# nanoporetech/scrappie

Measured on AMD Instinct MI355X. Metric: raw samples/sec, rgrgr_r94 4k-sample reads, higher is better.
Workload: dtype f32 (3xf16 split products, 22-bit operands, fp32 accumulate)

## Files before the change

include/scrappie_hip.h:

```cpp
#ifndef SCRAPPIE_HIP_H
#define SCRAPPIE_HIP_H

#include <stdbool.h>
#include <stddef.h>
#include <stdint.h>

#ifdef __cplusplus
extern "C" {
#endif


typedef struct {
    char *uuid;
    size_t n;
    size_t start;
    size_t end;
    float *raw;
} raw_table;

typedef struct {
    uint64_t start;
    float length;
    float mean;
    float stdv;
// ... 209 lines not shown

scrappie_matrix scrappie_hip_posterior(scrappie_hip_engine *e, int model, const raw_table signal,
                                       float min_prob, float tempW, float tempb, bool return_log);
scrappie_matrix scrappie_hip_trunk(scrappie_hip_engine *e, int model, const raw_table signal, int upto);

int scrappie_hip_event_features(const event_table events, float *out);
scrappie_matrix scrappie_hip_events_posterior(scrappie_hip_engine *e, int model, const float *feature3, size_t nevent,
                                              float min_prob, float tempW, float tempb, bool return_log);

long scrappie_hip_gru_schedule(const int *tile_T, size_t ntile, int ncu, int *nwg, int *capacity,
                               int *lane_off, int *seg, size_t cap);
long scrappie_hip_lane_schedule(const int *tile_T, size_t ntile, int ncu, int lanes_per_wg, int *nwg, int *capacity,
                                int *lane_off, int *seg, size_t cap);

long scrappie_hip_decoder_pieces(const int *tile_T, size_t ntile, int ncu, int *seg, size_t cap);

size_t scrappie_hip_min_samples(scrappie_hip_engine *e, int model);
int scrappie_hip_model_stride(scrappie_hip_engine *e, int model);
void scrappie_hip_set_profiling(scrappie_hip_engine *e, int on);
int scrappie_hip_get_timing(scrappie_hip_engine *e, scrappie_hip_timing *t);
void scrappie_hip_set_max_launch_reads(scrappie_hip_engine *e, size_t n);
void scrappie_hip_set_max_launch_blocks(scrappie_hip_engine *e, size_t n);
long scrappie_hip_plan_groups(const uint32_t *lengths, size_t n, int stride, size_t max_reads, size_t max_blocks,
                              size_t *starts, size_t cap);
unsigned scrappie_hip_host_thread_budget(void);
unsigned scrappie_hip_host_cpu_budget(void);
void *scrappie_hip_device_alloc(scrappie_hip_engine *e, size_t nbytes);
void scrappie_hip_device_free(scrappie_hip_engine *e, void *dptr);
int scrappie_hip_memcpy_h2d(scrappie_hip_engine *e, void *dst, const void *src, size_t nbytes);
int scrappie_hip_synchronize(scrappie_hip_engine *e);
// ... 18 lines not shown
```

scrappie_amd/csrc/scrappie_hip.hip:

```cpp
#include <hip/hip_runtime.h>
#include <sched.h>

#include <algorithm>
#include <atomic>
#include <cmath>
#include <cstdarg>
#include <cstdio>
#include <cstdlib>
#include <cstring>
#include <mutex>
#include <numeric>
#include <string>
#include <thread>
#include <vector>
#include <chrono>
#include <condition_variable>
#include <deque>
#include <map>
#include <memory>

#include "scrappie_hip.h"
#include "sh_internal.h"
#include "sh_kernels.h"
#include "sh_sched.h"
// ... 104 lines not shown
    std::vector<int> order;
    std::vector<int> rT, rN;
    std::vector<long long> seq_off, hp_off, bases_off;
    long long nbases_cap = 0;
    bool dev_stitch = false;
    bool dev_pos = false;
    int model = -1;
    bool hp_on = false;
    bool valid = false;
    int gru_nwg = 0;
    int gru1_nwg = 0;
    bool gru_two = false;
    int gru32_nwg = 0;
    int gru32x2_nwg = 0;
    int vit_nwg = 0;
    const float *d_signal = nullptr;
    std::vector<uint64_t> in_off;
    std::vector<uint32_t> in_len;
    scrappie_hip_params params{};
};

struct BatchReq {
    scrappie_hip_engine *e = nullptr;
    int model = 0;
    const raw_table *reads = nullptr;
    size_t n = 0;
    scrappie_hip_params p{};
    scrappie_hip_call *out = nullptr;
    int rc = -1;
    std::string err;
// ... 260 lines not shown
```

scrappie_amd/csrc/sh_decode.h:

```cpp
#ifndef SH_DECODE_H
#define SH_DECODE_H

struct ShVitArgs {
    const float *E;
    const float *sums;
    long long strideT;
    int strideQ, strideB;
    int want_log;
    float min_prob, stay_pen, skip_pen, local_pen;
    int use_slip;
    unsigned *tb;
    int *tb_end;
    int *final_state;
    float *final_score;
    float *hp_side;
    const long long *hp_off;
    unsigned long long *dbg;
    const ShGruSegD *seg;
    float *vstate;
    unsigned *flag;
    unsigned *err;
    int dump_final;
};

__device__ __forceinline__ void argmax_merge(float &v, int &i, float ov, int oi) {
    const bool take = (ov > v) | ((ov == v) & (oi < i));
    v = take ? ov : v;
    i = take ? oi : i;
}

__device__ __forceinline__ void rows_argmax(float &bv, int &bi) {
    float ov = __shfl_xor(bv, 16); int oi = __shfl_xor(bi, 16);
    argmax_merge(bv, bi, ov, oi);
// ... 949 lines not shown
```

scrappie_amd/csrc/sh_decode_teams.h:

```cpp
#ifndef SH_DECODE_TEAMS_H
#define SH_DECODE_TEAMS_H

#ifndef SH_FVT_WBUF
#define SH_FVT_WBUF 3
#endif
#ifndef SH_FVT_PROD_PRIO
#define SH_FVT_PROD_PRIO 1
#endif
#ifndef SH_FVT_ABL
#define SH_FVT_ABL 0
#endif
#ifndef SH_FVT_FLIP
#define SH_FVT_FLIP 3
#endif
#ifndef SH_FVT_STAMP
#ifdef SH_EXPERIMENTS
#define SH_FVT_STAMP 1
#else
#define SH_FVT_STAMP 0
#endif
#endif
#define SH_FVT_NTH 768
#define SH_FVT_LDS_FLOATS (1024 * 16 + 64 * 256 + 2 * 64 * 16 + 2 * 2 * 8 * 16 + 4 * 9 * 16 + 65 * 16 + 2 * 3 * 512 + 3 * 2 * 4 * 4)

template <bool SKIP0, bool DIV, bool NOCLAMP = false>
__global__ __launch_bounds__(SH_FVT_NTH) void k_ff_viterbi_teams(ShFfArgs f, ShVitArgs a, ShMeta md) {
    static_assert(!(DIV && NOCLAMP), "with temperatures the clamp stays");
    constexpr int NCW = 8, NPW = 4, PPT = 8, NQ = 256, NH = 1024, KS = 3, KQ = 6, TPP = 16, HT = 8, NG = 9, WB = SH_FVT_WBUF;
    static_assert(SH_SUM_GROUP == HT, "half a pass of a producer is one row-sum group");
    static_assert(WB >= 2 && WB <= 4, "weight ring");
    extern __shared__ __attribute__((aligned(16))) float smem[];
    float *sc = smem;
    float *ring = sc + NH * 16;
    float *skk = ring + 64 * 256;
    float *redv = skk + 2 * 64 * 16;
    int *redi = (int *)(redv + 2 * NCW * 16);
    float *gsum = (float *)(redi + 2 * NCW * 16);
    float *sBias = gsum + 4 * NG * 16;
    unsigned *xp = (unsigned *)(sBias + 65 * 16);
    unsigned *sStay = xp + 2 * KS * 512;

    const int tid = threadIdx.x, lane = tid & 63, b = lane & 15, q = lane >> 4;
    const int wave = __builtin_amdgcn_readfirstlane(tid >> 6);
    const bool decoder = wave < NCW;
    const float mp = a.min_prob, mpm1 = 1.0f - a.min_prob;
    const float lbound = (mp > 0.0f) ? 1.0e-3f - __logf(mp) : INFINITY;
    unsigned long long vA = 0, vB = 0, vC = 0, vD = 0, vt0 = 0, vt1 = 0;
    (void)vt0; (void)vt1;
#undef VSTAMP
#if SH_FVT_STAMP
#define VSTAMP(acc) do { if (a.dbg) { vt1 = __builtin_readcyclecounter(); acc += vt1 - vt0; vt0 = vt1; } } while (0)
#else
#define VSTAMP(acc) do { } while (0)
#endif

    if (tid < KS * 2 * 4 * 4) sStay[tid] = f.wpiece[(long long)(64) * KS * 512 + (tid >> 4) * 256 + ((tid >> 2) & 3) * 64 + (tid & 3)];
    for (int j = tid; j < 65 * 16; j += SH_FVT_NTH) sBias[j] = f.bfrag[((j >> 4) * 64 + ((j >> 2) & 3) * 16) * 4 + (j & 3)];

    int tile = blockIdx.x, s0 = 0, s1 = -1, ord = 0;
    if (a.seg) { const ShGruSegD sg = a.seg[blockIdx.x]; tile = sg.tile; s0 = sg.s0; s1 = sg.s1; ord = sg.pad; }
    tile = __builtin_amdgcn_readfirstlane(tile); s0 = __builtin_amdgcn_readfirstlane(s0); s1 = __builtin_amdgcn_readfirstlane(s1);
    const int Tt = __builtin_amdgcn_readfirstlane(md.tile_T[tile]);
    if (s1 < 0) s1 = Tt;
    const long long boff = __builtin_amdgcn_readfirstlane((int)md.tile_boff[tile]);
    const int rd = tile * 16 + b;
    int myT = md.rT[rd];
    asm volatile("" : "+v"(myT));
    const long long hpo = a.hp_side ? a.hp_off[rd] : 0;
    float pstart = 0.0f, pend = -SH_BIG;

    const int cw = decoder ? wave : 0;
    float *myq = sc + cw * 256 + lane * 4;
    const float *mye = ring + cw * 512 + lane * 4;
    const float *mysrc = sc + cw * 64 + b * 4 + q;
#define SH_FVT_MT(i) (16 * ((i) >> 1) + 8 * ((i) & 1))

    if (s0 == 0) {
        if (decoder) {
#pragma unroll
            for (int i = 0; i < PPT; i++) *(f32x4 *)(myq + SH_FVT_MT(i) * 256) = (f32x4){-SH_BIG, -SH_BIG, -SH_BIG, -SH_BIG};
            if (lane < 16) { redv[wave * 16 + b] = -SH_BIG - a.local_pen; redi[wave * 16 + b] = 4 * wave; }
        }
    } else {
        if (tid == 0) {
            if (!sh_wait_flag(a.flag + tile, (unsigned)ord, a.err)) __hip_atomic_store(a.err, 1u, __ATOMIC_RELAXED, __HIP_MEMORY_SCOPE_AGENT);
        }
        __syncthreads();
        __builtin_amdgcn_fence(__ATOMIC_ACQUIRE, "agent");
        if (decoder) {
            const float *vst = a.vstate + (long long)tile * (NH * 16 + 32);
            float bv = -INFINITY;
            int bi = 0x7fffffff;
#pragma unroll
            for (int i = 0; i < PPT; i++) {
                const int Q = 4 * (SH_FVT_MT(i) + cw) + q;
                const f32x4 pv = *(const f32x4 *)(vst + (Q * 16 + b) * 4);
                *(f32x4 *)(myq + SH_FVT_MT(i) * 256) = pv;
                {
                    const float ve = __builtin_fmaxf(__builtin_fmaxf(pv[0], pv[1]), __builtin_fmaxf(pv[2], pv[3])) - a.local_pen;
                    bi = (ve > bv) ? Q : bi;
                    bv = __builtin_fmaxf(bv, ve);
                }
            }
            pstart = vst[NH * 16 + b];
            pend = vst[NH * 16 + 16 + b];
// ... 149 lines not shown
            lds_barrier();
            VSTAMP(vD);
            if (more) w_prime(HT);
            VSTAMP(vA);
            lds_barrier();
            VSTAMP(vB);
            if (more) s1_half(H1, t + 2);
            __builtin_amdgcn_sched_barrier(0);
            xraw_load(t + 4);
            VSTAMP(vC);
            lds_barrier();
            VSTAMP(vD);
        }
        __syncthreads();
        if (s1 >= Tt) __syncthreads();
        if (a.dbg && lane == 0) { unsigned long long *d = a.dbg + ((long long)blockIdx.x * 12 + wave) * 8; d[0] = vA; d[1] = vB; d[2] = vC; d[3] = vD; d[4] = (unsigned long long)(s1 - s0); }
        return;
    }
    {
        f32x4 eN[2][PPT];
        auto drain = [&](auto a0, auto s0c, auto a1, auto s1c) {
            constexpr int A0 = decltype(a0)::value, S0 = decltype(s0c)::value, A1 = decltype(a1)::value, S1 = decltype(s1c)::value;
#pragma unroll
            for (int rl = 0; rl < PPT / 2; rl++) { eN[A0][2 * rl + S0] = *(const f32x4 *)(mye + rl * 4096); eN[A1][2 * rl + S1] = *(const f32x4 *)(mye + rl * 4096 + 256); }
        };
        const std::integral_constant<int, 0> I0{};
        const std::integral_constant<int, 1> I1{};
        __syncthreads();
        lds_barrier();
        lds_barrier();
        drain(I0, I0, I1, I0);
        lds_barrier();
        lds_barrier();
        if (a.dbg) vt0 = __builtin_readcyclecounter();
        const unsigned tofs = (unsigned)lane;
// ... 75 lines not shown
            const float rmf = d_rcp(tot) * mpm1;
            const float stay_lp = fin_log(gsum[((t & 3) * NG + NG - 1) * 16 + b], rmf, mp);
            const bool active = t < myT;
            const unsigned long long actmask = __builtin_amdgcn_ballot_w64(active);
            if (a.hp_side && active && tid < 16) (a.hp_side + (hpo + t) * 5)[4] = stay_lp;
            const float rm = active ? rmf : 0.0f;
            const float mpx = active ? mp : 0.0f;
            const float stay_v = active ? stay_lp - a.stay_pen : 0.0f;
            const float stay_act = stay_lp - a.stay_pen;
            const float hold = fmaxf(-a.local_pen, stay_act);
            const float nstart = pstart + hold;
            if (cw == 0) {
                float nend = pend + hold;
                const bool enter_end = ev > nend;
                nend = enter_end ? ev : nend;
                if (active && tid < 16) a.tb_end[cb * 16 + b] = enter_end ? tbe_in : NH + 1;
                if (active) pend = nend;
            }
            float bv = -INFINITY;
            int bi = 0x7fffffff;
            f32x4 pv_n; f32x2 kk_n;
            auto q_fetch = [&](int i) {
                pv_n = *(const f32x4 *)(myq + SH_FVT_MT(i) * 256);
                kk_n = *(const f32x2 *)(skk + ((SH_FVT_MT(i) + cw) * 16 + b) * 2);
            };
            q_fetch(0);
            float hpv[4] = {0.f, 0.f, 0.f, 0.f};
#pragma unroll
            for (int i = 0; i < PPT; i++) {
                const int QB = 4 * (SH_FVT_MT(i) + cw);
                const int Q = QB + q;
// ... 79 lines not shown
            }
            VSTAMP(vC);
            lds_barrier();
            VSTAMP(vD);
        };
        for (int t = s0; t < s1; t += 2) {
            block(t, std::true_type{});
            block(t + 1, std::false_type{});
#pragma unroll
            for (int rl = 0; rl < PPT / 2; rl++) eN[1][2 * rl] = eN[0][2 * rl + 1];
        }
    }

    if (s1 < Tt) {
        if (decoder) {
            float *vst = a.vstate + (long long)tile * (NH * 16 + 32);
#pragma unroll
            for (int i = 0; i < PPT; i++) {
                const int Q = 4 * (SH_FVT_MT(i) + cw) + q;
                *(f32x4 *)(vst + (Q * 16 + b) * 4) = *(const f32x4 *)(myq + SH_FVT_MT(i) * 256);
            }
            if (tid < 16) { vst[NH * 16 + b] = pstart; vst[NH * 16 + 16 + b] = pend; }
        }
        __builtin_amdgcn_fence(__ATOMIC_RELEASE, "agent");
        __syncthreads();
        if (tid == 0) __hip_atomic_store(a.flag + tile, (unsigned)ord + 1u, __ATOMIC_RELEASE, __HIP_MEMORY_SCOPE_AGENT);
    } else {
        float bv = -INFINITY;
        int bi = 0x7fffffff;
        if (decoder) {
#pragma unroll
            for (int i = 0; i < PPT; i++) {
                const int Q = 4 * (SH_FVT_MT(i) + cw) + q;
                const f32x4 pv = *(const f32x4 *)(myq + SH_FVT_MT(i) * 256);
#pragma unroll
                for (int k = 0; k < 4; k++) argmax_merge(bv, bi, pv[k], 4 * Q + k);
            }
            float ov = __shfl_xor(bv, 16); int oi = __shfl_xor(bi, 16);
            argmax_merge(bv, bi, ov, oi);
            ov = __shfl_xor(bv, 32); oi = __shfl_xor(bi, 32);
            argmax_merge(bv, bi, ov, oi);
        }
        __syncthreads();
        if (decoder && lane < 16) { redv[wave * 16 + b] = bv; redi[wave * 16 + b] = bi; }
        __syncthreads();
        if (tid < 16) {
            float ev = redv[b]; int ei = redi[b];
            for (int w = 1; w < NCW; w++) argmax_merge(ev, ei, redv[w * 16 + b], redi[w * 16 + b]);
            if (pstart > ev) { ev = pstart; ei = NH; }
            if (pend > ev) { ev = pend; ei = NH + 1; }
            a.final_state[rd] = ei;
            a.final_score[rd] = ev;
        }
        if (a.dump_final && a.vstate && decoder) {
            float *vst = a.vstate + (long long)tile * (NH * 16 + 32);
#pragma unroll
            for (int i = 0; i < PPT; i++) {
                const int Q = 4 * (SH_FVT_MT(i) + cw) + q;
                *(f32x4 *)(vst + (Q * 16 + b) * 4) = *(const f32x4 *)(myq + SH_FVT_MT(i) * 256);
            }
            if (tid < 16) { vst[NH * 16 + b] = pstart; vst[NH * 16 + 16 + b] = pend; }
        }
    }
    if (a.dbg && lane == 0) { unsigned long long *d = a.dbg + ((long long)blockIdx.x * 12 + wave) * 8; d[0] = vA; d[1] = vB; d[2] = vC; d[3] = vD; d[4] = (unsigned long long)(s1 - s0); }
#undef VSTAMP
#undef SH_FVT_MT
}

#endif
```

scrappie_amd/csrc/sh_eng_launch.inc:

```

struct MetaPtrs { ShMeta md; const long long *seq_off, *hp_off, *bases_off; ShGruLanes lanes, lanes1; ShGruPairs pairs, pairs2; const ShGruSegD *vseg; };

static int build_group(scrappie_hip_engine *e, Slot &sl, Model *m, const uint64_t *offsets, const uint32_t *lengths,
                       size_t n, bool hp_on, MetaPtrs &mp) {
    LaunchGroup &lg = sl.lg;
    lg.valid = false;
    lg.n = n; lg.hp_on = hp_on;
    lg.ntile = (n + 15) / 16; lg.npad = lg.ntile * 16;
    const int st = m->stride;
    std::vector<int> T(n);
    for (size_t i = 0; i < n; i++)
        T[i] = (lengths[i] >= m->min_samples) ? (int)((lengths[i] + st - 1) / st) : 0;
    lg.order.assign(lg.npad, -1);
    std::vector<int> idx(n);
    std::iota(idx.begin(), idx.end(), 0);
    std::stable_sort(idx.begin(), idx.end(), [&](int a, int b) { return T[a] > T[b]; });
    for (size_t i = 0; i < n; i++) lg.order[i] = idx[i];
    lg.rT.assign(lg.npad, 0); lg.rN.assign(lg.npad, 0);
    lg.seq_off.assign(lg.npad, 0); lg.hp_off.assign(lg.npad, 0); lg.bases_off.assign(lg.npad, 0);
    long long nbases = 0;
    const long long per_entry = (m->arch == 1) ? 1 : 5;
    std::vector<unsigned long long> sig_off(lg.npad, 0);
    std::vector<int> tile_T(lg.ntile, 0);
    std::vector<long long> tile_boff(lg.ntile, 0);
// ... 26 lines not shown
      if (e->dbg_gru_tiles == 1) lg.gru_two = false;
      if (e->dbg_gru_tiles == 2 && tmax < 65536) lg.gru_two = true; }
    std::vector<int> pair_tile, pair_T;
    for (size_t t = 0; t < lg.ntile; ) {
        const bool two = t + 1 < lg.ntile && tile_T[t] < (1 << 18) && tile_T[t + 1] > 0;
        pair_tile.push_back((int)t); pair_tile.push_back(two ? (int)t + 1 : -1);
        pair_T.push_back(std::max(tile_T[t], two ? tile_T[t + 1] : 0));
        t += two ? 2 : 1;
    }
    ShGruSchedule sched32;
    sh_lane_schedule(pair_T.data(), pair_T.size(), e->ncu, 1, sched32, e->handover);
    lg.gru32_nwg = sched32.nwg;
    ShGruSchedule sched32b;
    sh_lane_schedule(pair_T.data(), pair_T.size(), e->ncu, 2, sched32b, e->handover);
    lg.gru32x2_nwg = sched32b.nwg;
    std::vector<ShGruSeg> vseg;
    sh_piece_schedule(tile_T.data(), lg.ntile, e->ncu, vseg, e->handover);
    lg.vit_nwg = (int)vseg.size();
    const size_t b_u64 = lg.npad * 8, b_i32 = lg.npad * 4;
    const size_t b_loff = sched.lane_off.size() * 4, b_seg = sched.seg.size() * sizeof(ShGruSeg), b_wit = sched.wg_iter.size() * 4;
    const size_t b_vloff = 0, b_vseg = vseg.size() * sizeof(ShGruSeg);
    const size_t b_loff1 = sched1.lane_off.size() * 4, b_seg1 = sched1.seg.size() * sizeof(ShGruSeg);
    const size_t b_loff32 = sched32.lane_off.size() * 4, b_seg32 = sched32.seg.size() * sizeof(ShGruSeg), b_pt = pair_tile.size() * 4;
    const size_t b_loff32b = sched32b.lane_off.size() * 4, b_seg32b = sched32b.seg.size() * sizeof(ShGruSeg);
    const size_t total = 4 * b_u64 + lg.ntile * 8 + 2 * b_i32 + lg.ntile * 4 + 16 + b_seg + b_loff + b_wit + 16 + b_vseg + b_vloff + 16 + b_seg1 + b_loff1 +
                         16 + b_seg32 + b_loff32 + b_pt + 16 + b_seg32b + b_loff32b;
    if (sl.h_meta.ensure(total + 16) || sl.d_meta.ensure(total + 16)) return -1;
    char *h = sl.h_meta.as<char>();
    size_t o = 0;
    memcpy(h + o, sig_off.data(), b_u64); const size_t o_sig = o; o += b_u64;
    memcpy(h + o, lg.seq_off.data(), b_u64); const size_t o_seq = o; o += b_u64;
    memcpy(h + o, lg.hp_off.data(), b_u64); const size_t o_hp = o; o += b_u64;
    memcpy(h + o, lg.bases_off.data(), b_u64); const size_t o_bs = o; o += b_u64;
    memcpy(h + o, tile_boff.data(), lg.ntile * 8); const size_t o_tb = o; o += lg.ntile * 8;
    memcpy(h + o, lg.rN.data(), b_i32); const size_t o_n = o; o += b_i32;
    memcpy(h + o, lg.rT.data(), b_i32); const size_t o_t = o; o += b_i32;
    memcpy(h + o, tile_T.data(), lg.ntile * 4); const size_t o_tt = o; o += lg.ntile * 4;
    o = (o + 15) & ~(size_t)15;
    memcpy(h + o, sched.seg.data(), b_seg); const size_t o_seg = o; o += b_seg;
    memcpy(h + o, sched.lane_off.data(), b_loff); const size_t o_loff = o; o += b_loff;
    memcpy(h + o, sched.wg_iter.data(), b_wit); const size_t o_wit = o; o += b_wit;
    o = (o + 15) & ~(size_t)15;
    memcpy(h + o, vseg.data(), b_vseg); const size_t o_vseg = o; o += b_vseg;
    o = (o + 15) & ~(size_t)15;
    memcpy(h + o, sched1.seg.data(), b_seg1); const size_t o_seg1 = o; o += b_seg1;
    memcpy(h + o, sched1.lane_off.data(), b_loff1); const size_t o_loff1 = o; o += b_loff1;
    o = (o + 15) & ~(size_t)15;
    memcpy(h + o, sched32.seg.data(), b_seg32); const size_t o_seg32 = o; o += b_seg32;
    memcpy(h + o, sched32.lane_off.data(), b_loff32); const size_t o_loff32 = o; o += b_loff32;
    memcpy(h + o, pair_tile.data(), b_pt); const size_t o_pt = o; o += b_pt;
    o = (o + 15) & ~(size_t)15;
    memcpy(h + o, sched32b.seg.data(), b_seg32b); const size_t o_seg32b = o; o += b_seg32b;
    memcpy(h + o, sched32b.lane_off.data(), b_loff32b); const size_t o_loff32b = o; o += b_loff32b;
    hipStream_t ps = e->ev_ok ? e->pstream : e->stream;
    if (e->ev_ok) {
        const long long n16 = (long long)((total + 15) / 16);
        hipLaunchKernelGGL(k_upload_words, dim3((unsigned)std::min<long long>((n16 + 255) / 256, 64)), dim3(256), 0, ps, (const u32x4 *)h, sl.d_meta.as<u32x4>(), n16);
    } else HIPCHK(hipMemcpyAsync(sl.d_meta.p, h, total, hipMemcpyHostToDevice, ps));
    char *d = sl.d_meta.as<char>();
    mp.md.sig_off = (const unsigned long long *)(d + o_sig);
    mp.seq_off = (const long long *)(d + o_seq);
    mp.hp_off = (const long long *)(d + o_hp);
    mp.bases_off = (const long long *)(d + o_bs);
    mp.md.tile_boff = (const long long *)(d + o_tb);
    mp.md.rN = (const int *)(d + o_n);
    mp.md.rT = (const int *)(d + o_t);
    mp.md.tile_T = (const int *)(d + o_tt);
    static_assert(sizeof(ShGruSeg) == sizeof(ShGruSegD), "segment layout");
    mp.lanes.seg = (const ShGruSegD *)(d + o_seg);
    mp.lanes.lane_off = (const int *)(d + o_loff);
    mp.lanes.wg_iter = (const int *)(d + o_wit);
    mp.lanes.ntile = (int)lg.ntile;
    mp.vseg = (const ShGruSegD *)(d + o_vseg);
    if (e->d_hstate.ensure(std::max<size_t>(lg.ntile, 1) * 12 * 256 * 4) || sl.d_gflag.ensure((lg.ntile + 1) * 4)) return -1;
    mp.lanes.hstate = e->d_hstate.as<float>();
    mp.lanes.flag = sl.d_gflag.as<unsigned>();
    HIPCHK(hipMemsetAsync(sl.d_gflag.p, 0, (lg.ntile + 1) * 4, ps));
    if (sl.d_bad.ensure(lg.npad * 4)) return -1;
    HIPCHK(hipMemsetAsync(sl.d_bad.p, 0, lg.npad * 4, ps));
    mp.lanes1 = mp.lanes;
    mp.lanes1.seg = (const ShGruSegD *)(d + o_seg1);
    mp.lanes1.lane_off = (const int *)(d + o_loff1);
    mp.lanes1.wg_iter = nullptr;
    mp.pairs.seg = (const ShGruSegD *)(d + o_seg32);
    mp.pairs.lane_off = (const int *)(d + o_loff32);
    mp.pairs.pair_tile = (const int *)(d + o_pt);
    mp.pairs.hstate = mp.lanes.hstate;
    mp.pairs.flag = mp.lanes.flag;
// ... 650 lines not shown
    case 64: VIT_CASE(256, 1) break;
    case 256: VIT_CASE(256, 4) break;
    case 1024:
#ifdef SH_EXPERIMENTS
        if (getenv("SH_VIT_1024")) { VIT_CASE(1024, 4) break; }
#endif
        VIT_CASE(512, 8) break;
    default: return set_err("unsupported transducer state count %d (need 4^3, 4^4 or 4^5 k-mers)", NH);
    }
#undef VIT_CASE1
#undef VIT_CASE2
#undef VIT_CASE
    return 0;
}

static int launch_ff_viterbi(hipStream_t s, const ShFfArgs &f, const ShVitArgs &a, const ShMeta &md, size_t nwg, bool single) {
    const size_t lds = (size_t)SH_FV_LDS_FLOATS * 4;
    if (nwg == 0) return 0;
    dim3 grid((unsigned)nwg);
    if (!a.use_slip && !single) {
        const size_t ldt = (size_t)SH_FVT_LDS_FLOATS * 4;
#define FVT_CASE(SK0, DIV, NC)                                                                                    \
    {                                                                                                             \
        static DevOnce attr_once;                                                                                 \
        if (auto turn_ = attr_once.first())                                                                                    \
            HIPCHK(hipFuncSetAttribute((const void *)k_ff_viterbi_teams<SK0, DIV, NC>, hipFuncAttributeMaxDynamicSharedMemorySize, (int)ldt)); \
        hipLaunchKernelGGL((k_ff_viterbi_teams<SK0, DIV, NC>), grid, dim3(SH_FVT_NTH), ldt, s, f, a, md);         \
    }
        const bool skip0 = a.skip_pen == 0.0f, dv = f.out_div != 1.0f || f.in_div != 1.0f;
        static const bool keep_clamp = getenv("SH_FVT_KEEP_CLAMP") != nullptr;
        const bool nc = f.no_clamp && !dv && !keep_clamp;
        if (skip0) { if (dv) FVT_CASE(true, true, false) else if (nc) FVT_CASE(true, false, true) else FVT_CASE(true, false, false) }
        else { if (dv) FVT_CASE(false, true, false) else if (nc) FVT_CASE(false, false, true) else FVT_CASE(false, false, false) }
#undef FVT_CASE
        return 0;
    }
// ... 14 lines not shown
```

scrappie_amd/csrc/sh_eng_load.inc:

```

static const HostMat *find_mat(const std::vector<std::pair<std::string, HostMat>> &ms, const char *nm) {
    for (auto &kv : ms) if (kv.first == nm) return &kv.second;
    return nullptr;
}

static int load_model_mem_one(scrappie_hip_engine *e, const char *name, const void *blob, size_t nbytes);
extern "C" int scrappie_hip_load_model_mem(scrappie_hip_engine *e, const char *name, const void *blob, size_t nbytes) {
    const int idx = load_model_mem_one(e, name, blob, nbytes);
    if (idx < 0 || e->is_tail) return idx;
    scrappie_hip_engine::Blob b{name, std::vector<unsigned char>((const unsigned char *)blob, (const unsigned char *)blob + nbytes), e->dbg_force_f32};
    bool found = false;
    for (auto &x : e->blobs) if (x.name == b.name) { x = b; found = true; }
    if (!found) e->blobs.push_back(b);
    if (e->tail || e->tail2) {
        std::unique_lock<std::mutex> lk(e->tail_mu);
        e->tail_cv.wait(lk, [&] { return e->tail_busy == 0 && e->tail_q.empty(); });
    }
    for (scrappie_hip_engine **tp : {&e->tail, &e->tail2}) if (*tp) {
        (*tp)->dbg_force_f32 = e->dbg_force_f32;
        if (load_model_mem_one(*tp, name, blob, nbytes) != idx) return set_err("model '%s' did not load at the same index on the helper engine", name);
    }
    return idx;
}
static int load_model_mem_one(scrappie_hip_engine *e, const char *name, const void *blob, size_t nbytes) {
// ... 277 lines not shown
}

extern "C" long scrappie_hip_gru_schedule(const int *tile_T, size_t ntile, int ncu, int *nwg, int *capacity,
                                          int *lane_off, int *seg, size_t cap) {
    return scrappie_hip_lane_schedule(tile_T, ntile, ncu, 2, nwg, capacity, lane_off, seg, cap);
}

extern "C" long scrappie_hip_decoder_pieces(const int *tile_T, size_t ntile, int ncu, int *seg, size_t cap) {
    if (!tile_T || ncu < 1) return -1;
    std::vector<ShGruSeg> v;
    sh_piece_schedule(tile_T, ntile, ncu, v);
    if (seg) for (size_t i = 0; i < v.size() && i < cap; i++) memcpy(seg + 4 * i, &v[i], 16);
    return (long)v.size();
}

extern "C" long scrappie_hip_plan_groups(const uint32_t *lengths, size_t n, int stride, size_t max_reads, size_t max_blocks,
                                         size_t *starts, size_t cap) {
    if ((!lengths && n) || stride < 1 || max_reads < 1) return -1;
    long ng = 0;
    size_t cnt = 0;
    unsigned long long sumT = 0, maxT = 0;
    for (size_t i = 0; i < n; i++) {
        const unsigned long long T = ((unsigned long long)lengths[i] + stride - 1) / stride;
        if (max_blocks && T / 16 + T + 1 > max_blocks) return -1;
        const unsigned long long ns = sumT + T, nm = std::max(maxT, T);
        if (cnt == 0 || cnt >= max_reads || (max_blocks && ns / 16 + nm + 1 > max_blocks)) {
            if (starts && (size_t)ng < cap) starts[ng] = i;
            ng++;
            cnt = 0; sumT = 0; maxT = 0;
        }
// ... 25 lines not shown
```

scrappie_amd/csrc/sh_eng_pipeline.inc:

```

enum StopAt { STOP_NONE = 0, STOP_TRUNK = 1, STOP_POST = 2 };

struct RunOut {
    const float *act = nullptr;
    int act_units = 0;
    const float *E = nullptr;
    const float *sums = nullptr;
};

struct HostStamp {
    const std::chrono::steady_clock::time_point t0 = std::chrono::steady_clock::now();
    void operator()(const char *what, const char *after = "") const {
        if (tun().host_stamp) fprintf(stderr, "host stamp: %s %.2f ms%s\n", what, std::chrono::duration<double, std::milli>(std::chrono::steady_clock::now() - t0).count(), after);
    }
};

struct Marks {
    enum Mark { PROLOGUE_BEGIN, PROLOGUE_END,
                WAIT_BEGIN, MAIN_BEGIN,
                LAYER_BEGIN, LAYER_SPLIT, LAYER_END,
                S1_BEGIN, S1_END, DECODE_END, MAIN_END,
                WALK_BEGIN, WALK_END, STITCH_BEGIN, STITCH_END,
                N_MARKS };
    Slot *sl = nullptr;
// ... 242 lines not shown
    const int NH = m->NS - 1, NQ = NH / 4;
    if (e->d_tb.ensure((size_t)ncb * NQ * 16 * 4) || e->d_tbend.ensure((size_t)ncb * 16 * 4) || e->d_fstate.ensure(lg.npad * 4)) return -1;
    if (c.hp_on && sl.d_hp.ensure((size_t)std::max<long long>(lg.nhp, 1) * 5 * 4)) return -1;
    ShVitArgs va;
    va.E = E_use; va.sums = sums_use;
    va.strideT = (long long)mtiles * 256; va.strideQ = 64; va.strideB = 4;
    va.want_log = 1; va.min_prob = p->min_prob;
    va.stay_pen = p->stay_pen; va.skip_pen = p->skip_pen; va.local_pen = p->local_pen; va.use_slip = p->use_slip;
    va.tb = e->d_tb.as<unsigned>(); va.tb_end = e->d_tbend.as<int>();
    va.final_state = e->d_fstate.as<int>(); va.final_score = sl.d_fscore.as<float>();
    va.hp_side = c.hp_on ? sl.d_hp.as<float>() : nullptr; va.hp_off = mp.hp_off;
    va.dbg = nullptr;
    va.dump_final = e->dbg_dump_final ? 1 : 0;
    static unsigned long long *vdbg = nullptr;
    if (tun().vit_stamp) { if (!vdbg) (void)hipMalloc(&vdbg, 4096 * 16 * 8 * 8); va.dbg = vdbg; }
    if (e->d_vstate.ensure(std::max<size_t>(lg.ntile, 1) * ((size_t)NH * 16 + 32) * 4) || e->d_vflag.ensure(std::max<size_t>(lg.ntile, 1) * 4)) return -1;
    HIPCHK(hipMemsetAsync(e->d_vflag.p, 0, std::max<size_t>(lg.ntile, 1) * 4, s));
    va.seg = mp.vseg;
    va.vstate = e->d_vstate.as<float>(); va.flag = e->d_vflag.as<unsigned>(); va.err = sl.d_gflag.as<unsigned>() + lg.ntile;
    if (e->ev_ok && e->other(sl).pending) HIPCHK(hipStreamWaitEvent(s, e->other(sl).done, 0));
    if (fused) {
        ShFfArgs fa;
        fa.in = top; fa.wpiece = m->ffWp.as<unsigned>(); fa.bfrag = m->ffbs.as<float>();
        fa.in_div = p->tempW / p->tempb; fa.out_div = p->tempb;
        fa.no_clamp = (m->ff_no_clamp && !e->alt_trunk) ? 1 : 0;
        va.E = nullptr; va.sums = nullptr;
        if (launch_ff_viterbi(s, fa, va, mp.md, (size_t)lg.vit_nwg, tun().fv_single || e->dbg_fv_single)) return -1;
    } else if (launch_viterbi(s, NH, va, mp.md, (size_t)lg.vit_nwg)) return -1;
    if (va.dbg) {
        (void)sh_stream_wait(s);
        std::vector<unsigned long long> h((size_t)std::max(lg.vit_nwg, 1) * 16 * 8);
        (void)hipMemcpy(h.data(), vdbg, h.size() * 8, hipMemcpyDeviceToHost);
        const int nwv = (fused && !va.use_slip && !(tun().fv_single || e->dbg_fv_single)) ? 12 : 8;
        for (int w = 0; w < nwv; w++) { unsigned long long *d = &h[((size_t)(lg.vit_nwg / 2) * nwv + w) * 8]; fprintf(stderr, "vit stamp wave %d: phaseB %.0f bar %.0f phaseC %.0f bar %.0f cycles/block\n", w, d[0] / (double)d[4], d[1] / (double)d[4], d[2] / (double)d[4], d[3] / (double)d[4]); }
    }
    if (c.pf.mark(Marks::DECODE_END, s)) return -1;
    c.pf.span(F_DECODE, Marks::S1_END, Marks::DECODE_END);
    c.stamp("decoder enqueued at");
    c.walk_on_cs = e->ev_ok;
    if (c.walk_on_cs) { HIPCHK(hipEventRecord(sl.kdone, s)); HIPCHK(hipStreamWaitEvent(e->cstream, sl.kdone, 0)); }
    c.fold_tail = c.walk_on_cs && !tun().split_tail && !tun().host_stitch;
    if (!c.fold_tail) {
        hipStream_t bs = c.walk_on_cs ? e->cstream : s;
        if (c.pf.mark(Marks::WALK_BEGIN, bs)) return -1;
        hipLaunchKernelGGL(k_backtrace, dim3((unsigned)((lg.npad + 63) / 64)), dim3(64), 0, bs, e->d_tb.as<unsigned>(), e->d_tbend.as<int>(),
                           e->d_fstate.as<int>(), mp.md, mp.seq_off, sl.d_seq.as<int>(), (int)lg.npad, NQ, SH_SEQ_STRIDE);
        if (c.pf.mark(Marks::WALK_END, bs)) return -1;
        c.pf.span(F_BACKTRACE, Marks::WALK_BEGIN, Marks::WALK_END);
    }
// ... 143 lines not shown
```

scrappie_amd/csrc/sh_eng_surface.inc:

```

struct PostReq {
    int model = -1;
    raw_table sig{};
    float min_prob = 0.f, tempW = 1.f, tempb = 1.f;
    bool want_log = true;
    StopAt stop = STOP_POST;
    int upto = 5;
    scrappie_matrix out = nullptr;
    size_t nr = 0, nc = 0;
    const float *src = nullptr;
    size_t nbytes = 0;
    std::atomic<int> *users = nullptr;
    int phase = 0;
    char err[256] = "";
};
static void post_fail(PostReq *r, const char *fmt, ...) {
    va_list ap;
    va_start(ap, fmt);
    vsnprintf(r->err, sizeof r->err, fmt, ap);
    va_end(ap);
}
static void posterior_batch(scrappie_hip_engine *e, std::vector<PostReq *> &reqs) {
    if (reqs.empty()) return;
    Model *m = get_model(e, reqs[0]->model);
// ... 301 lines not shown
        char *d = dmeta.as<char>();
        ShMeta md;
        md.sig_off = (const unsigned long long *)d;
        md.tile_boff = (const long long *)(d + npad * 24);
        md.rN = (const int *)(d + npad * 24 + n * 8);
        md.rT = md.rN + npad;
        md.tile_T = md.rT + npad;
        ShVitArgs va;
        va.E = dpost.as<float>(); va.sums = nullptr;
        va.strideT = (long long)stride; va.strideQ = 4; va.strideB = 0;
        va.want_log = 0; va.min_prob = 0.f;
        va.stay_pen = f->stay_pen; va.skip_pen = f->skip_pen; va.local_pen = f->local_pen; va.use_slip = f->slip ? 1 : 0;
        va.tb = dtb.as<unsigned>(); va.tb_end = dtbe.as<int>();
        va.final_state = dfs.as<int>(); va.final_score = dfsc.as<float>();
        va.hp_side = nullptr; va.hp_off = nullptr; va.dbg = nullptr; va.dump_final = 0;
        va.seg = nullptr; va.vstate = nullptr; va.flag = nullptr; va.err = nullptr;
        if (launch_viterbi(s, NH, va, md, n)) break;
        hipLaunchKernelGGL(k_backtrace_lane0, dim3((unsigned)((n + 63) / 64)), dim3(64), 0, s, dtb.as<unsigned>(), dtbe.as<int>(), dfs.as<int>(), md,
                           (const long long *)(d + npad * 8), dseq.as<int>(), (int)n, NQ);
        int *hseq = e->h_dec_out.as<int>();
        if (hipMemcpyAsync(hseq, dseq.p, (size_t)nseq * 4, hipMemcpyDeviceToHost, s) != hipSuccess) break;
        if (hipMemcpyAsync(hseq + nseq, dfsc.p, npad * 4, hipMemcpyDeviceToHost, s) != hipSuccess) break;
        if (sh_stream_wait(s) != hipSuccess) break;
        const float *hsc = (const float *)(hseq + nseq);
        for (size_t k = 0; k < n; k++) {
            memcpy(reqs[k]->seq, hseq + seq_off[k * 16], ((size_t)reqs[k]->post->nc + 1) * 4);
            reqs[k]->score = hsc[k * 16];
        }
        ok = true;
    } while (0);
    if (!ok) { (void)hipGetLastError(); for (DecReq *r : reqs) r->score = NAN; }
// ... 160 lines not shown
```

scrappie_amd/csrc/sh_sched.h:

```cpp
#ifndef SH_SCHED_H
#define SH_SCHED_H
#include <algorithm>
#include <vector>

struct ShGruSeg { int tile, s0, s1, pad; };

struct ShGruSchedule {
    int nwg = 0;
    int capacity = 0;
    std::vector<int> lane_off;
    std::vector<ShGruSeg> seg;
    std::vector<int> wg_iter;
};

static inline void sh_lane_schedule(const int *tile_T, size_t ntile, int ncu, int lpw, ShGruSchedule &out,
                                    bool allow_split = true) {
    out = ShGruSchedule();
    std::vector<int> live;
    long long W = 0;
    int maxT = 0;
    for (size_t t = 0; t < ntile; t++) if (tile_T[t] > 0) { live.push_back((int)t); W += tile_T[t]; maxT = std::max(maxT, tile_T[t]); }
    if (live.empty()) { out.lane_off.assign(1, 0); return; }
    const long long nlive = (long long)live.size();
    const int nwg = (int)std::min<long long>(ncu, nlive);
// ... 38 lines not shown
    }
    out.nwg = nwg; out.capacity = M;
    out.lane_off.assign(L + 1, 0);
    out.wg_iter.assign(nwg, 0);
    for (int ln = 0; ln < L; ln++) {
        const std::vector<ShGruSeg> &v = pos[L - 1 - ln];
        int steps = 0;
        for (const ShGruSeg &sg : v) { out.seg.push_back(sg); steps += sg.s1 - sg.s0; }
        out.lane_off[ln + 1] = (int)out.seg.size();
        out.wg_iter[ln / lpw] = std::max(out.wg_iter[ln / lpw], steps);
    }
}
static inline void sh_gru_schedule(const int *tile_T, size_t ntile, int ncu, ShGruSchedule &out) {
    sh_lane_schedule(tile_T, ntile, ncu, 2, out);
}

static inline int sh_pieces_per_tile(long long nlive, int ncu) {
    if (nlive <= ncu) return 1;
    int best = 1;
    double bestv = 1e30;
    for (int k = 1; k <= 4; k++) {
        const double v = (double)((nlive * k + ncu - 1) / ncu) / k;
        if (v < bestv - 1e-9) { bestv = v; best = k; }
    }
    return best;
}
static inline void sh_piece_schedule(const int *tile_T, size_t ntile, int ncu, std::vector<ShGruSeg> &seg,
                                     bool allow_split = true) {
    seg.clear();
    long long nlive = 0;
// ... 13 lines not shown
```

Baseline: 1.582 billion.

## Make fused FF-Viterbi teams decoder persistent with per-CU lane schedule

```diff
diff --git a/include/scrappie_hip.h b/include/scrappie_hip.h
--- a/include/scrappie_hip.h
+++ b/include/scrappie_hip.h
@@ -247,6 +247,7 @@
                                 int *lane_off, int *seg, size_t cap);
 
 long scrappie_hip_decoder_pieces(const int *tile_T, size_t ntile, int ncu, int *seg, size_t cap);
+long scrappie_hip_decoder_lanes(const int *tile_T, size_t ntile, int ncu, int *nwg, int *capacity, int *lane_off, int *seg, size_t cap);
 
 size_t scrappie_hip_min_samples(scrappie_hip_engine *e, int model);
 int scrappie_hip_model_stride(scrappie_hip_engine *e, int model);
diff --git a/scrappie_amd/csrc/scrappie_hip.hip b/scrappie_amd/csrc/scrappie_hip.hip
--- a/scrappie_amd/csrc/scrappie_hip.hip
+++ b/scrappie_amd/csrc/scrappie_hip.hip
@@ -142,6 +142,7 @@
     int gru32_nwg = 0;
     int gru32x2_nwg = 0;
     int vit_nwg = 0;
+    int vit_npiece = 0;
     const float *d_signal = nullptr;
     std::vector<uint64_t> in_off;
     std::vector<uint32_t> in_len;
diff --git a/scrappie_amd/csrc/sh_decode.h b/scrappie_amd/csrc/sh_decode.h
--- a/scrappie_amd/csrc/sh_decode.h
+++ b/scrappie_amd/csrc/sh_decode.h
@@ -17,6 +17,7 @@
     const long long *hp_off;
     unsigned long long *dbg;
     const ShGruSegD *seg;
+    const int *lane_off;
     float *vstate;
     unsigned *flag;
     unsigned *err;
diff --git a/scrappie_amd/csrc/sh_decode_teams.h b/scrappie_amd/csrc/sh_decode_teams.h
--- a/scrappie_amd/csrc/sh_decode_teams.h
+++ b/scrappie_amd/csrc/sh_decode_teams.h
@@ -22,6 +22,8 @@
 #endif
 #define SH_FVT_NTH 768
 #define SH_FVT_LDS_FLOATS (1024 * 16 + 64 * 256 + 2 * 64 * 16 + 2 * 2 * 8 * 16 + 4 * 9 * 16 + 65 * 16 + 2 * 3 * 512 + 3 * 2 * 4 * 4)
+
+struct ShFvtKernArgs { ShFfArgs f; ShVitArgs a; ShMeta md; };
 
 template <bool SKIP0, bool DIV, bool NOCLAMP = false>
 __global__ __launch_bounds__(SH_FVT_NTH) void k_ff_viterbi_teams(ShFfArgs f, ShVitArgs a, ShMeta md) {
@@ -40,12 +42,13 @@
     unsigned *xp = (unsigned *)(sBias + 65 * 16);
     unsigned *sStay = xp + 2 * KS * 512;
 
-    const int tid = threadIdx.x, lane = tid & 63, b = lane & 15, q = lane >> 4;
-    const int wave = __builtin_amdgcn_readfirstlane(tid >> 6);
+    const int tid0 = threadIdx.x;
+    const int wave = __builtin_amdgcn_readfirstlane(tid0 >> 6);
     const bool decoder = wave < NCW;
     const float mp = a.min_prob, mpm1 = 1.0f - a.min_prob;
     const float lbound = (mp > 0.0f) ? 1.0e-3f - __logf(mp) : INFINITY;
     unsigned long long vA = 0, vB = 0, vC = 0, vD = 0, vt0 = 0, vt1 = 0;
+    int vblocks = 0;
     (void)vt0; (void)vt1;
 #undef VSTAMP
 #if SH_FVT_STAMP
@@ -54,26 +57,37 @@
 #define VSTAMP(acc) do { } while (0)
 #endif
 
-    if (tid < KS * 2 * 4 * 4) sStay[tid] = f.wpiece[(long long)(64) * KS * 512 + (tid >> 4) * 256 + ((tid >> 2) & 3) * 64 + (tid & 3)];
-    for (int j = tid; j < 65 * 16; j += SH_FVT_NTH) sBias[j] = f.bfrag[((j >> 4) * 64 + ((j >> 2) & 3) * 16) * 4 + (j & 3)];
-
-    int tile = blockIdx.x, s0 = 0, s1 = -1, ord = 0;
-    if (a.seg) { const ShGruSegD sg = a.seg[blockIdx.x]; tile = sg.tile; s0 = sg.s0; s1 = sg.s1; ord = sg.pad; }
-    tile = __builtin_amdgcn_readfirstlane(tile); s0 = __builtin_amdgcn_readfirstlane(s0); s1 = __builtin_amdgcn_readfirstlane(s1);
-    const int Tt = __builtin_amdgcn_readfirstlane(md.tile_T[tile]);
-    if (s1 < 0) s1 = Tt;
-    const long long boff = __builtin_amdgcn_readfirstlane((int)md.tile_boff[tile]);
-    const int rd = tile * 16 + b;
-    int myT = md.rT[rd];
-    asm volatile("" : "+v"(myT));
-    const long long hpo = a.hp_side ? a.hp_off[rd] : 0;
-    float pstart = 0.0f, pend = -SH_BIG;
-
+    if (tid0 < KS * 2 * 4 * 4) sStay[tid0] = f.wpiece[(long long)(64) * KS * 512 + (tid0 >> 4) * 256 + ((tid0 >> 2) & 3) * 64 + (tid0 & 3)];
+    for (int j = tid0; j < 65 * 16; j += SH_FVT_NTH) sBias[j] = f.bfrag[((j >> 4) * 64 + ((j >> 2) & 3) * 16) * 4 + (j & 3)];
+
+#define SH_FVT_MT(i) (16 * ((i) >> 1) + 8 * ((i) & 1))
+
+    int sgi = blockIdx.x, sgn = blockIdx.x + 1;
+    if (a.lane_off) { sgi = a.lane_off[blockIdx.x]; sgn = a.lane_off[blockIdx.x + 1]; }
+    sgi = __builtin_amdgcn_readfirstlane(sgi); sgn = __builtin_amdgcn_readfirstlane(sgn);
+    auto segment = [&](auto dec_c, const int sgi) __attribute__((always_inline)) {
+    constexpr bool decoder = decltype(dec_c)::value;
     const int cw = decoder ? wave : 0;
+    typedef const __attribute__((address_space(4))) ShFvtKernArgs *kargs_t;
+    kargs_t ka = (kargs_t)__builtin_amdgcn_kernarg_segment_ptr();
+    asm volatile("" : "+s"(ka));
+    int lane;
+    asm volatile("v_mbcnt_lo_u32_b32 %0, -1, 0\n\tv_mbcnt_hi_u32_b32 %0, -1, %0" : "=v"(lane));
+    const int tid = wave * 64 + lane, b = lane & 15, q = lane >> 4;
     float *myq = sc + cw * 256 + lane * 4;
     const float *mye = ring + cw * 512 + lane * 4;
     const float *mysrc = sc + cw * 64 + b * 4 + q;
-#define SH_FVT_MT(i) (16 * ((i) >> 1) + 8 * ((i) & 1))
+    int tile = sgi, s0 = 0, s1 = -1, ord = 0;
+    if (ka->a.seg) { const ShGruSegD sg = ka->a.seg[sgi]; tile = sg.tile; s0 = sg.s0; s1 = sg.s1; ord = sg.pad; }
+    tile = __builtin_amdgcn_readfirstlane(tile); s0 = __builtin_amdgcn_readfirstlane(s0); s1 = __builtin_amdgcn_readfirstlane(s1);
+    const int Tt = __builtin_amdgcn_readfirstlane(ka->md.tile_T[tile]);
+    if (s1 < 0) s1 = Tt;
+    const long long boff = __builtin_amdgcn_readfirstlane((int)ka->md.tile_boff[tile]);
+    const int rd = tile * 16 + b;
+    int myT = ka->md.rT[rd];
+    asm volatile("" : "+v"(myT));
+    const long long hpo = a.hp_side ? ka->a.hp_off[rd] : 0;
+    float pstart = 0.0f, pend = -SH_BIG;
 
     if (s0 == 0) {
         if (decoder) {
@@ -83,12 +97,12 @@
         }
     } else {
         if (tid == 0) {
-            if (!sh_wait_flag(a.flag + tile, (unsigned)ord, a.err)) __hip_atomic_store(a.err, 1u, __ATOMIC_RELAXED, __HIP_MEMORY_SCOPE_AGENT);
+            if (!sh_wait_flag(ka->a.flag + tile, (unsigned)ord, ka->a.err)) __hip_atomic_store(ka->a.err, 1u, __ATOMIC_RELAXED, __HIP_MEMORY_SCOPE_AGENT);
         }
         __syncthreads();
         __builtin_amdgcn_fence(__ATOMIC_ACQUIRE, "agent");
         if (decoder) {
-            const float *vst = a.vstate + (long long)tile * (NH * 16 + 32);
+            const float *vst = ka->a.vstate + (long long)tile * (NH * 16 + 32);
             float bv = -INFINITY;
             int bi = 0x7fffffff;
 #pragma unroll
@@ -268,11 +282,12 @@
         }
         __syncthreads();
         if (s1 >= Tt) __syncthreads();
-        if (a.dbg && lane == 0) { unsigned long long *d = a.dbg + ((long long)blockIdx.x * 12 + wave) * 8; d[0] = vA; d[1] = vB; d[2] = vC; d[3] = vD; d[4] = (unsigned long long)(s1 - s0); }
+        vblocks += s1 - s0;
+        __syncthreads();
         return;
     }
     {
-        f32x4 eN[2][PPT];
+        f32x4 eN[2][PPT] = {};
         auto drain = [&](auto a0, auto s0c, auto a1, auto s1c) {
             constexpr int A0 = decltype(a0)::value, S0 = decltype(s0c)::value, A1 = decltype(a1)::value, S1 = decltype(s1c)::value;
 #pragma unroll
@@ -378,7 +393,11 @@
                 float nend = pend + hold;
                 const bool enter_end = ev > nend;
                 nend = enter_end ? ev : nend;
-                if (active && tid < 16) a.tb_end[cb * 16 + b] = enter_end ? tbe_in : NH + 1;
+                if (active && tid < 16) {
+                    unsigned bo = (unsigned)b;
+                    asm volatile("" : "+v"(bo));
+                    (a.tb_end + cb * 16)[bo] = enter_end ? tbe_in : NH + 1;
+                }
                 if (active) pend = nend;
             }
             float bv = -INFINITY;
@@ -488,7 +507,7 @@
 
     if (s1 < Tt) {
         if (decoder) {
-            float *vst = a.vstate + (long long)tile * (NH * 16 + 32);
+            float *vst = ka->a.vstate + (long long)tile * (NH * 16 + 32);
 #pragma unroll
             for (int i = 0; i < PPT; i++) {
                 const int Q = 4 * (SH_FVT_MT(i) + cw) + q;
@@ -498,7 +517,7 @@
         }
         __builtin_amdgcn_fence(__ATOMIC_RELEASE, "agent");
         __syncthreads();
-        if (tid == 0) __hip_atomic_store(a.flag + tile, (unsigned)ord + 1u, __ATOMIC_RELEASE, __HIP_MEMORY_SCOPE_AGENT);
+        if (tid == 0) __hip_atomic_store(ka->a.flag + tile, (unsigned)ord + 1u, __ATOMIC_RELEASE, __HIP_MEMORY_SCOPE_AGENT);
     } else {
         float bv = -INFINITY;
         int bi = 0x7fffffff;
@@ -523,11 +542,11 @@
             for (int w = 1; w < NCW; w++) argmax_merge(ev, ei, redv[w * 16 + b], redi[w * 16 + b]);
             if (pstart > ev) { ev = pstart; ei = NH; }
             if (pend > ev) { ev = pend; ei = NH + 1; }
-            a.final_state[rd] = ei;
-            a.final_score[rd] = ev;
-        }
-        if (a.dump_final && a.vstate && decoder) {
-            float *vst = a.vstate + (long long)tile * (NH * 16 + 32);
+            ka->a.final_state[rd] = ei;
+            ka->a.final_score[rd] = ev;
+        }
+        if (ka->a.dump_final && ka->a.vstate && decoder) {
+            float *vst = ka->a.vstate + (long long)tile * (NH * 16 + 32);
 #pragma unroll
             for (int i = 0; i < PPT; i++) {
                 const int Q = 4 * (SH_FVT_MT(i) + cw) + q;
@@ -536,7 +555,12 @@
             if (tid < 16) { vst[NH * 16 + b] = pstart; vst[NH * 16 + 16 + b] = pend; }
         }
     }
-    if (a.dbg && lane == 0) { unsigned long long *d = a.dbg + ((long long)blockIdx.x * 12 + wave) * 8; d[0] = vA; d[1] = vB; d[2] = vC; d[3] = vD; d[4] = (unsigned long long)(s1 - s0); }
+    vblocks += s1 - s0;
+    __syncthreads();
+    };
+    if (decoder) { for (; sgi < sgn; sgi++) segment(std::true_type{}, sgi); }
+    else { for (; sgi < sgn; sgi++) segment(std::false_type{}, sgi); }
+    if (a.dbg && __builtin_amdgcn_mbcnt_hi(~0u, __builtin_amdgcn_mbcnt_lo(~0u, 0u)) == 0) { unsigned long long *d = a.dbg + ((long long)blockIdx.x * 12 + wave) * 8; d[0] = vA; d[1] = vB; d[2] = vC; d[3] = vD; d[4] = (unsigned long long)vblocks; }
 #undef VSTAMP
 #undef SH_FVT_MT
 }
diff --git a/scrappie_amd/csrc/sh_eng_launch.inc b/scrappie_amd/csrc/sh_eng_launch.inc
--- a/scrappie_amd/csrc/sh_eng_launch.inc
+++ b/scrappie_amd/csrc/sh_eng_launch.inc
@@ -1,5 +1,5 @@
 
-struct MetaPtrs { ShMeta md; const long long *seq_off, *hp_off, *bases_off; ShGruLanes lanes, lanes1; ShGruPairs pairs, pairs2; const ShGruSegD *vseg; };
+struct MetaPtrs { ShMeta md; const long long *seq_off, *hp_off, *bases_off; ShGruLanes lanes, lanes1; ShGruPairs pairs, pairs2; const ShGruSegD *vseg, *vlseg; const int *vlane_off; };
 
 static int build_group(scrappie_hip_engine *e, Slot &sl, Model *m, const uint64_t *offsets, const uint32_t *lengths,
                        size_t n, bool hp_on, MetaPtrs &mp) {
@@ -64,16 +64,19 @@
     ShGruSchedule sched32b;
     sh_lane_schedule(pair_T.data(), pair_T.size(), e->ncu, 2, sched32b, e->handover);
     lg.gru32x2_nwg = sched32b.nwg;
+    ShGruSchedule vsched;
+    sh_decoder_lanes(tile_T.data(), lg.ntile, e->ncu, vsched, e->handover);
+    lg.vit_nwg = vsched.nwg;
     std::vector<ShGruSeg> vseg;
     sh_piece_schedule(tile_T.data(), lg.ntile, e->ncu, vseg, e->handover);
-    lg.vit_nwg = (int)vseg.size();
+    lg.vit_npiece = (int)vseg.size();
     const size_t b_u64 = lg.npad * 8, b_i32 = lg.npad * 4;
     const size_t b_loff = sched.lane_off.size() * 4, b_seg = sched.seg.size() * sizeof(ShGruSeg), b_wit = sched.wg_iter.size() * 4;
-    const size_t b_vloff = 0, b_vseg = vseg.size() * sizeof(ShGruSeg);
+    const size_t b_vseg = vseg.size() * sizeof(ShGruSeg), b_vloff = vsched.lane_off.size() * 4, b_vlseg = vsched.seg.size() * sizeof(ShGruSeg);
     const size_t b_loff1 = sched1.lane_off.size() * 4, b_seg1 = sched1.seg.size() * sizeof(ShGruSeg);
     const size_t b_loff32 = sched32.lane_off.size() * 4, b_seg32 = sched32.seg.size() * sizeof(ShGruSeg), b_pt = pair_tile.size() * 4;
     const size_t b_loff32b = sched32b.lane_off.size() * 4, b_seg32b = sched32b.seg.size() * sizeof(ShGruSeg);
-    const size_t total = 4 * b_u64 + lg.ntile * 8 + 2 * b_i32 + lg.ntile * 4 + 16 + b_seg + b_loff + b_wit + 16 + b_vseg + b_vloff + 16 + b_seg1 + b_loff1 +
+    const size_t total = 4 * b_u64 + lg.ntile * 8 + 2 * b_i32 + lg.ntile * 4 + 16 + b_seg + b_loff + b_wit + 16 + b_vseg + b_vlseg + b_vloff + 16 + b_seg1 + b_loff1 +
                          16 + b_seg32 + b_loff32 + b_pt + 16 + b_seg32b + b_loff32b;
     if (sl.h_meta.ensure(total + 16) || sl.d_meta.ensure(total + 16)) return -1;
     char *h = sl.h_meta.as<char>();
@@ -92,6 +95,8 @@
     memcpy(h + o, sched.wg_iter.data(), b_wit); const size_t o_wit = o; o += b_wit;
     o = (o + 15) & ~(size_t)15;
     memcpy(h + o, vseg.data(), b_vseg); const size_t o_vseg = o; o += b_vseg;
+    memcpy(h + o, vsched.seg.data(), b_vlseg); const size_t o_vlseg = o; o += b_vlseg;
+    memcpy(h + o, vsched.lane_off.data(), b_vloff); const size_t o_vloff = o; o += b_vloff;
     o = (o + 15) & ~(size_t)15;
     memcpy(h + o, sched1.seg.data(), b_seg1); const size_t o_seg1 = o; o += b_seg1;
     memcpy(h + o, sched1.lane_off.data(), b_loff1); const size_t o_loff1 = o; o += b_loff1;
@@ -122,6 +127,8 @@
     mp.lanes.wg_iter = (const int *)(d + o_wit);
     mp.lanes.ntile = (int)lg.ntile;
     mp.vseg = (const ShGruSegD *)(d + o_vseg);
+    mp.vlseg = (const ShGruSegD *)(d + o_vlseg);
+    mp.vlane_off = (const int *)(d + o_vloff);
     if (e->d_hstate.ensure(std::max<size_t>(lg.ntile, 1) * 12 * 256 * 4) || sl.d_gflag.ensure((lg.ntile + 1) * 4)) return -1;
     mp.lanes.hstate = e->d_hstate.as<float>();
     mp.lanes.flag = sl.d_gflag.as<unsigned>();
@@ -802,12 +809,13 @@
     return 0;
 }
 
-static int launch_ff_viterbi(hipStream_t s, const ShFfArgs &f, const ShVitArgs &a, const ShMeta &md, size_t nwg, bool single) {
+static int launch_ff_viterbi(hipStream_t s, const ShFfArgs &f, const ShVitArgs &a, const ShMeta &md, size_t nwg, bool single, int ncu) {
     const size_t lds = (size_t)SH_FV_LDS_FLOATS * 4;
     if (nwg == 0) return 0;
     dim3 grid((unsigned)nwg);
     if (!a.use_slip && !single) {
         const size_t ldt = (size_t)SH_FVT_LDS_FLOATS * 4;
+        if (a.lane_off && nwg > (size_t)ncu) return set_err("decoder: %zu persistent workgroups for %d CUs", nwg, ncu);
 #define FVT_CASE(SK0, DIV, NC)                                                                                    \
     {                                                                                                             \
         static DevOnce attr_once;                                                                                 \
diff --git a/scrappie_amd/csrc/sh_eng_load.inc b/scrappie_amd/csrc/sh_eng_load.inc
--- a/scrappie_amd/csrc/sh_eng_load.inc
+++ b/scrappie_amd/csrc/sh_eng_load.inc
@@ -315,6 +315,18 @@
     return (long)v.size();
 }
 
+extern "C" long scrappie_hip_decoder_lanes(const int *tile_T, size_t ntile, int ncu, int *nwg, int *capacity, int *lane_off,
+                                           int *seg, size_t cap) {
+    if (!tile_T || ncu < 1) return -1;
+    ShGruSchedule sc;
+    sh_decoder_lanes(tile_T, ntile, ncu, sc);
+    if (nwg) *nwg = sc.nwg;
+    if (capacity) *capacity = sc.capacity;
+    if (lane_off) memcpy(lane_off, sc.lane_off.data(), sc.lane_off.size() * sizeof(int));
+    if (seg) for (size_t i = 0; i < sc.seg.size() && i < cap; i++) memcpy(seg + 4 * i, &sc.seg[i], 16);
+    return (long)sc.seg.size();
+}
+
 extern "C" long scrappie_hip_plan_groups(const uint32_t *lengths, size_t n, int stride, size_t max_reads, size_t max_blocks,
                                          size_t *starts, size_t cap) {
     if ((!lengths && n) || stride < 1 || max_reads < 1) return -1;
diff --git a/scrappie_amd/csrc/sh_eng_pipeline.inc b/scrappie_amd/csrc/sh_eng_pipeline.inc
--- a/scrappie_amd/csrc/sh_eng_pipeline.inc
+++ b/scrappie_amd/csrc/sh_eng_pipeline.inc
@@ -280,9 +280,12 @@
     va.dump_final = e->dbg_dump_final ? 1 : 0;
     static unsigned long long *vdbg = nullptr;
     if (tun().vit_stamp) { if (!vdbg) (void)hipMalloc(&vdbg, 4096 * 16 * 8 * 8); va.dbg = vdbg; }
+    const bool teams = fused && !va.use_slip && !(tun().fv_single || e->dbg_fv_single);
+    const int vit_nwg = teams ? lg.vit_nwg : lg.vit_npiece;
     if (e->d_vstate.ensure(std::max<size_t>(lg.ntile, 1) * ((size_t)NH * 16 + 32) * 4) || e->d_vflag.ensure(std::max<size_t>(lg.ntile, 1) * 4)) return -1;
     HIPCHK(hipMemsetAsync(e->d_vflag.p, 0, std::max<size_t>(lg.ntile, 1) * 4, s));
-    va.seg = mp.vseg;
+    va.seg = teams ? mp.vlseg : mp.vseg;
+    va.lane_off = teams ? mp.vlane_off : nullptr;
     va.vstate = e->d_vstate.as<float>(); va.flag = e->d_vflag.as<unsigned>(); va.err = sl.d_gflag.as<unsigned>() + lg.ntile;
     if (e->ev_ok && e->other(sl).pending) HIPCHK(hipStreamWaitEvent(s, e->other(sl).done, 0));
     if (fused) {
@@ -291,14 +294,14 @@
         fa.in_div = p->tempW / p->tempb; fa.out_div = p->tempb;
         fa.no_clamp = (m->ff_no_clamp && !e->alt_trunk) ? 1 : 0;
         va.E = nullptr; va.sums = nullptr;
-        if (launch_ff_viterbi(s, fa, va, mp.md, (size_t)lg.vit_nwg, tun().fv_single || e->dbg_fv_single)) return -1;
-    } else if (launch_viterbi(s, NH, va, mp.md, (size_t)lg.vit_nwg)) return -1;
+        if (launch_ff_viterbi(s, fa, va, mp.md, (size_t)vit_nwg, !teams, e->ncu)) return -1;
+    } else if (launch_viterbi(s, NH, va, mp.md, (size_t)vit_nwg)) return -1;
     if (va.dbg) {
         (void)sh_stream_wait(s);
-        std::vector<unsigned long long> h((size_t)std::max(lg.vit_nwg, 1) * 16 * 8);
+        std::vector<unsigned long long> h((size_t)std::max(vit_nwg, 1) * 16 * 8);
         (void)hipMemcpy(h.data(), vdbg, h.size() * 8, hipMemcpyDeviceToHost);
-        const int nwv = (fused && !va.use_slip && !(tun().fv_single || e->dbg_fv_single)) ? 12 : 8;
-        for (int w = 0; w < nwv; w++) { unsigned long long *d = &h[((size_t)(lg.vit_nwg / 2) * nwv + w) * 8]; fprintf(stderr, "vit stamp wave %d: phaseB %.0f bar %.0f phaseC %.0f bar %.0f cycles/block\n", w, d[0] / (double)d[4], d[1] / (double)d[4], d[2] / (double)d[4], d[3] / (double)d[4]); }
+        const int nwv = teams ? 12 : 8;
+        for (int w = 0; w < nwv; w++) { unsigned long long *d = &h[((size_t)(vit_nwg / 2) * nwv + w) * 8]; fprintf(stderr, "vit stamp wave %d: phaseB %.0f bar %.0f phaseC %.0f bar %.0f cycles/block\n", w, d[0] / (double)d[4], d[1] / (double)d[4], d[2] / (double)d[4], d[3] / (double)d[4]); }
     }
     if (c.pf.mark(Marks::DECODE_END, s)) return -1;
     c.pf.span(F_DECODE, Marks::S1_END, Marks::DECODE_END);
diff --git a/scrappie_amd/csrc/sh_eng_surface.inc b/scrappie_amd/csrc/sh_eng_surface.inc
--- a/scrappie_amd/csrc/sh_eng_surface.inc
+++ b/scrappie_amd/csrc/sh_eng_surface.inc
@@ -339,7 +339,7 @@
         va.tb = dtb.as<unsigned>(); va.tb_end = dtbe.as<int>();
         va.final_state = dfs.as<int>(); va.final_score = dfsc.as<float>();
         va.hp_side = nullptr; va.hp_off = nullptr; va.dbg = nullptr; va.dump_final = 0;
-        va.seg = nullptr; va.vstate = nullptr; va.flag = nullptr; va.err = nullptr;
+        va.seg = nullptr; va.lane_off = nullptr; va.vstate = nullptr; va.flag = nullptr; va.err = nullptr;
         if (launch_viterbi(s, NH, va, md, n)) break;
         hipLaunchKernelGGL(k_backtrace_lane0, dim3((unsigned)((n + 63) / 64)), dim3(64), 0, s, dtb.as<unsigned>(), dtbe.as<int>(), dfs.as<int>(), md,
                            (const long long *)(d + npad * 8), dseq.as<int>(), (int)n, NQ);
diff --git a/scrappie_amd/csrc/sh_sched.h b/scrappie_amd/csrc/sh_sched.h
--- a/scrappie_amd/csrc/sh_sched.h
+++ b/scrappie_amd/csrc/sh_sched.h
@@ -76,6 +76,10 @@
 static inline void sh_gru_schedule(const int *tile_T, size_t ntile, int ncu, ShGruSchedule &out) {
     sh_lane_schedule(tile_T, ntile, ncu, 2, out);
 }
+static inline void sh_decoder_lanes(const int *tile_T, size_t ntile, int ncu, ShGruSchedule &out, bool allow_split = true) {
+    sh_lane_schedule(tile_T, ntile, ncu, 1, out, allow_split);
+    for (ShGruSeg &sg : out.seg) sg.pad = sg.s0 > 0 ? 1 : 0;
+}
 
 static inline int sh_pieces_per_tile(long long nlive, int ncu) {
     if (nlive <= ncu) return 1;
```

Result: no change. 1.584 billion, median of 6 (+0.2%).
